# CristianSimion5/vk-raytracing-engine

Measured on AMD Instinct MI355X. Metric: Mrays/s, higher is better.
Workload: dtype f32

## Files before the change

vk-raytracing-engine_amd/csrc/traverse_share.h:

```cpp
#pragma once
#include "traverse_wide.h"

#define VKRT_SHARE_LDS_WORDS 384
struct ShareRes
{
  unsigned long long* key;
  int* slot;
  float* u;
  float* v;
  int* donor;
};
VKRT_DEV void shareSync()
{
  __builtin_amdgcn_fence(__ATOMIC_RELEASE, "wavefront");
  __builtin_amdgcn_wave_barrier();
  __builtin_amdgcn_fence(__ATOMIC_ACQUIRE, "wavefront");
}
VKRT_DEV unsigned laneRank(unsigned long long mask)
{
  return __builtin_amdgcn_mbcnt_hi((unsigned)(mask >> 32), __builtin_amdgcn_mbcnt_lo((unsigned)mask, 0u));
}
typedef unsigned vkrt_u32x2 __attribute__((ext_vector_type(2)));
typedef __attribute__((address_space(3))) vkrt_u32x2* ShareStk;
VKRT_DEV uint2 stkLoad(ShareStk p)
{
  const vkrt_u32x2 e = *p;
  return make_uint2(e.x, e.y);
}
VKRT_DEV void stkStore(ShareStk p, uint2 e)
{
  vkrt_u32x2 w;
  w.x = e.x; w.y = e.y;
  *p = w;
}
VKRT_DEV ShareRes shareRes(int* lds320)
{
  ShareRes r;
  r.key = (unsigned long long*)lds320; r.slot = lds320 + 128; r.u = (float*)(lds320 + 192); r.v = (float*)(lds320 + 256); r.donor = lds320 + 320;
  return r;
}

template <bool COUNT, bool ANYHIT, int TM = 0>
VKRT_DEV void traverse_wide8_share(const DevScene& sc, bool valid, f3 o, f3 d, float tmin, float tmax, uint2* stk, ShareRes res, RayHit& hit,
                                   TravCount& tc, uint32_t raySeed = 0u)
{
  TriRay<(TM & VKRT_TM_WATERTIGHT) != 0> tr;
  tr.set(d);
  const float4* __restrict__ nodes = sc.nodes;
  const float4* __restrict__ tris = sc.tris;
  const int stride = 64;
  const int lane = (int)lane_id();
  const ShareStk stkBase = (ShareStk)stk, stkCap = stkBase + (int)(sc.stackCap >> 1) * stride;
  const unsigned shareMin = sc.shareMinIdle;
  bool farFirst = ANYHIT && anyhit_far_first(sc, o, d, tmax);

  res.key[lane] = ((unsigned long long)__float_as_uint(tmax) << 32) | 0xffffffffull;
  res.slot[lane] = -1; res.u[lane] = 0.0f; res.v[lane] = 0.0f;
  shareSync();

  int owner = lane;
  unsigned long long* ownerKey = res.key + lane;
  int* ownerSlot = res.slot + lane;
  f3 id = mk3(safe_inv(d.x), safe_inv(d.y), safe_inv(d.z));
  bool px = !(id.x < 0.0f), py = !(id.y < 0.0f), pz = !(id.z < 0.0f);
  unsigned oct4 = ((px ? 1u : 0u) | (py ? 2u : 0u) | (pz ? 4u : 0u)) * 0x01010101u;
  uint2 G = make_uint2(0u, (valid && sc.rootRef != VKRT_TRAV_DONE) ? 0x80000000u : 0u);
  uint2 T = make_uint2(0u, 0u);
  ShareStk sp = stkBase, sb = stkBase, top = stkCap;
  bool busy = G.y != 0u;
  const unsigned iterLimit = sc.stepLimit > 0x03ffffffu ? 0xffffffffu : sc.stepLimit * 64u;
  const bool lendOn = (TM & (VKRT_TM_WATERTIGHT | VKRT_TM_DISSOLVE)) != (VKRT_TM_WATERTIGHT | VKRT_TM_DISSOLVE) && (sc.shareFlags & VKRT_SHARE_TRI_LEND) != 0u;

  for(unsigned iter = 0;; iter++)
  {
    const unsigned long long busyMask = __ballot(busy);
    if(busyMask == 0ull || iter >= iterLimit)
      break;
    if((iter & sc.sharePeriodMask) == sc.sharePeriodMask && (unsigned)__popcll(~busyMask) >= shareMin)
    {
      const bool giveStack = busy && sp > sb;
      const bool giveChild = (sc.shareFlags & 1u) != 0u && busy && !giveStack && (G.y & 0xff000000u & ((G.y & 0xff000000u) - 1u)) != 0u;
      const bool mayTris = (sc.shareFlags & 16u) != 0u && busy && !giveStack && !giveChild;
      const bool giveParked = mayTris && top < stkCap;
      const bool giveTris = mayTris && !giveParked && (T.y & (T.y - 1u)) != 0u;
      const bool wants = giveStack || giveChild || giveParked || giveTris;
      const unsigned long long donorMask = __ballot(wants), idleMask = ~busyMask;
      if(donorMask != 0ull)
      {
        const unsigned n = min((unsigned)__popcll(donorMask), (unsigned)__popcll(idleMask));
        const unsigned giveRank = laneRank(donorMask), takeRank = laneRank(idleMask);
        const bool gives = wants && giveRank < n;
        const bool takes = !busy && takeRank < n;
        uint2 e = make_uint2(0u, 0u);
        if(gives)
        {
          if(giveStack)
          {
            e = stkLoad(sb);
            sb += stride;
          }
          else if(giveChild)
          {
            const unsigned top = G.y & 0xff000000u;
            const unsigned low = farFirst ? (0x80000000u >> (unsigned)__clz((int)top)) : (top & (0u - top));
            e = make_uint2(G.x, low | (G.y & 0xffu));
            G.y &= ~low;
          }
          else if(giveParked)
          {
            e = stkLoad(top);
            e.x |= 0x80000000u;
            top += stride;
          }
          else
          {
            const unsigned lo = (unsigned)__ffs((int)T.y) - 1u, hi = 31u - (unsigned)__clz((int)T.y);
            const unsigned upper = T.y & ~((1u << ((lo + hi + 1u) >> 1)) - 1u);
            e = make_uint2(T.x | 0x80000000u, upper);
            T.y &= ~upper;
          }
          res.donor[giveRank] = lane;
        }
        shareSync();
        const int src = takes ? res.donor[takeRank] : lane;
        const unsigned ex = (unsigned)__shfl((int)e.x, src), ey = (unsigned)__shfl((int)e.y, src);
        const float ox = __shfl(o.x, src), oy = __shfl(o.y, src), oz = __shfl(o.z, src);
        const float dx = __shfl(d.x, src), dy = __shfl(d.y, src), dz = __shfl(d.z, src);
        const float ix = __shfl(id.x, src), iy = __shfl(id.y, src), iz = __shfl(id.z, src);
        const float tm = __shfl(tmax, src);
        const int ow = __shfl(owner, src);
        const unsigned o4 = (unsigned)__shfl((int)oct4, src);
        if(TM & VKRT_TM_DISSOLVE)
        {
          const uint32_t sd = (uint32_t)__shfl((int)raySeed, src);
          if(takes) raySeed = sd;
        }
        if(takes)
        {
          o = mk3(ox, oy, oz); d = mk3(dx, dy, dz); id = mk3(ix, iy, iz); tmax = tm;
          tr.set(d);
          farFirst = ANYHIT && anyhit_far_first(sc, o, d, tmax);
          px = !(id.x < 0.0f); py = !(id.y < 0.0f); pz = !(id.z < 0.0f);
          oct4 = o4;
          if(ex & 0x80000000u)
          {
            G = make_uint2(0u, 0u);
            T = make_uint2(ex & 0x7fffffffu, ey);
          }
          else
          {
            G = make_uint2(ex, ey);
            T = make_uint2(0u, 0u);
          }
          sp = stkBase; sb = stkBase; top = stkCap;
          owner = ow;
          ownerKey = res.key + ow; ownerSlot = res.slot + ow;
          busy = true;
        }
      }
    }
    shareSync();
    if(busy || lendOn)
    {
      float bt = tmax;
      int bg = -1;
      bool finished = false;
      bool occluded = false;
      if(ANYHIT)
        finished = busy && __hip_atomic_load(ownerSlot, __ATOMIC_RELAXED, __HIP_MEMORY_SCOPE_WAVEFRONT) >= 0;
      else
      {
        const unsigned long long k = __hip_atomic_load(ownerKey, __ATOMIC_RELAXED, __HIP_MEMORY_SCOPE_WAVEFRONT);
        bt = __uint_as_float((unsigned)(k >> 32));
        bg = (int)(unsigned)k;
      }
      if(!finished)
      {
        struct Cand
        {
          bool found;
          float t, u, v;
          int slot, gid;
        };
        auto testOne = [&](Cand& cd) {
          const unsigned i = (unsigned)__ffs((int)T.y) - 1u;
          T.y &= T.y - 1u;
          const unsigned s = T.x + i;
          const float4* __restrict__ tp = tris + (size_t)s * VKRT_TRI_QUADS;
          const float4 a = tp[0];
          const float4 b = tp[1];
          const float4 c = tp[2];
          if(COUNT)
          {
            tc.tris++;
            if(lane == __ffsll((long long)__ballot(1)) - 1) tc.waveTriSteps++;
          }
          float t, u, v;
          bool ccw;
          if(tr.hit(o, d, a, b, c, t, u, v, ccw) && t > tmin)
          {
            if(ANYHIT)
            {
              if(t < tmax && !cd.found && !query_rejects<TM>(sc, c, ccw) && !anyhit_ignores<TM>(sc, s, c.y, raySeed, VKRT_HOOK_UV(TM, u, v)))
              {
                cd.found = true; cd.t = t; cd.slot = (int)s;
              }
            }
            else
            {
              const int gid = tri_gid<TM>(c.y);
              const float rt = cd.found ? cd.t : bt;
              const int rg = cd.found ? cd.gid : bg;
              if((t < rt || (t == rt && gid < rg)) && !query_rejects<TM>(sc, c, ccw) && !anyhit_ignores<TM>(sc, s, c.y, raySeed, VKRT_HOOK_UV(TM, u, v)))
              {
                cd.found = true; cd.t = t; cd.u = u; cd.v = v; cd.slot = (int)s; cd.gid = gid;
              }
            }
          }
        };
        auto publish = [&](const Cand& cd) {
          if(!cd.found)
            return;
          if(ANYHIT)
          {
            __hip_atomic_store(ownerSlot, cd.slot, __ATOMIC_RELAXED, __HIP_MEMORY_SCOPE_WAVEFRONT);
            occluded = true;
          }
          else
          {
            const unsigned long long mine = ((unsigned long long)__float_as_uint(cd.t) << 32) | (unsigned)cd.gid;
            __hip_atomic_fetch_min(ownerKey, mine, __ATOMIC_RELAXED, __HIP_MEMORY_SCOPE_WAVEFRONT);
            shareSync();
            if(__hip_atomic_load(ownerKey, __ATOMIC_RELAXED, __HIP_MEMORY_SCOPE_WAVEFRONT) == mine)
            {
              res.slot[owner] = cd.slot; res.u[owner] = cd.u; res.v[owner] = cd.v;
            }
            bt = cd.t; bg = cd.gid;
          }
        };
        auto flushT = [&]() {
          Cand cd = {false, 0.0f, 0.0f, 0.0f, -1, 0};
          while(T.y != 0u && !(ANYHIT && cd.found))
            testOne(cd);
          publish(cd);
        };
        if(G.y & 0xff000000u)
        {
          const unsigned bitIdx = farFirst ? (unsigned)__ffs((int)(G.y & 0xff000000u)) - 1u : 31u - (unsigned)__clz((int)G.y);
          const unsigned slot = (bitIdx - 24u) ^ (oct4 & 7u);
          const unsigned child = G.x + (unsigned)__popc(G.y & 0xffu & ((1u << slot) - 1u));
          G.y &= ~(1u << bitIdx);
          if(G.y & 0xff000000u)
          {
            bool full = sp >= top;
            if(__builtin_expect(full && top < stkCap - VKRT_W8_POSTPONE_ROOM * stride, 0))
            {
              const uint2 keep = T;
              T = stkLoad(top);
              top += stride;
              flushT();
              T = keep;
              full = sp >= top;
            }
            if(!full)
            {
              stkStore(sp, G);
              sp += stride;
            }
            else
              VKRT_TRAV_FAULT(sc);
          }
          uint2 Tn;
          w8_test_children<COUNT, (TM & VKRT_TM_FILTER) != 0>(nodes, child, o, id, oct4, px, py, pz, tmin, bt, G, Tn, tc, query_node_masks<TM>(sc),
                                                              query_cull_mask<TM>(sc));
          if(Tn.y != 0u)
          {
            if(T.y != 0u)
            {
              if(__builtin_expect(top > stkCap - VKRT_W8_MAX_POSTPONED * stride && sp < top, 1))
              {
                top -= stride;
                stkStore(top, T);
              }
              else
              {
                if(!occluded)
                  flushT();
                T.y = 0u;
              }
            }
            T = Tn;
          }
        }
        if((G.y & 0xff000000u) == 0u && sp > sb)
        {
          sp -= stride;
          G = stkLoad(sp);
        }
        if(T.y == 0u && top < stkCap)
        {
          T = stkLoad(top);
          top += stride;
        }
        const unsigned long long hasTMask = __ballot(T.y != 0u);
        bool triStep = true;
        if(sc.triThreshold > 1u)
          triStep = (unsigned)__popcll(hasTMask) * 64u >= sc.triThreshold * (unsigned)__popcll(busyMask) ||
                    __ballot((G.y & 0xff000000u) != 0u) == 0ull;
        bool lentStep = false;
        if(lendOn && triStep)
        {
          const bool tests = T.y != 0u && !occluded;
          const unsigned rest1 = T.y & (T.y - 1u);
          const bool multi = rest1 != 0u && !occluded, isFree = T.y == 0u && !occluded;
          const unsigned long long lendMask = __ballot(multi), freeMask = ANYHIT ? __ballot(isFree) : (__ballot(true) & ~hasTMask);
          const unsigned n = min((unsigned)__popcll(lendMask), (unsigned)__popcll(freeMask));
          if(n != 0u)
          {
            lentStep = true;
            const unsigned lendRank = laneRank(lendMask), freeRank = laneRank(freeMask);
            const bool borrows = isFree && freeRank < n;
            unsigned s = 0u, ls = 0u;
            if(multi && lendRank < n)
            {
              const unsigned hi = 31u - (unsigned)__clz((int)T.y);
              T.y &= ~(1u << hi);
              ls = T.x + hi;
              res.donor[lendRank] = lane;
            }
            if(tests)
            {
              s = T.x + (unsigned)__ffs((int)T.y) - 1u;
              T.y &= T.y - 1u;
            }
            shareSync();
            const int src = borrows ? res.donor[freeRank] : lane;
            const unsigned bs = (unsigned)__shfl((int)ls, src);
            const f3 ro = mk3(__shfl(o.x, src), __shfl(o.y, src), __shfl(o.z, src));
            const f3 rd = mk3(__shfl(d.x, src), __shfl(d.y, src), __shfl(d.z, src));
            const int row = __shfl(owner, src);
            const float rbt = __shfl(bt, src);
            const int rbg = ANYHIT ? 0 : __shfl(bg, src);
            uint32_t rseed = raySeed;
            if(TM & VKRT_TM_DISSOLVE)
              rseed = (uint32_t)__shfl((int)raySeed, src);
            if(tests || borrows)
            {
              if(borrows)
              {
                s = bs;
                tr.set(rd);
              }
              const float4* __restrict__ tp = tris + (size_t)s * VKRT_TRI_QUADS;
              const float4 a = tp[0];
              const float4 b = tp[1];
              const float4 c = tp[2];
              if(COUNT)
              {
                tc.tris++;
                if(lane == __ffsll((long long)__ballot(1)) - 1) tc.waveTriSteps++;
              }
              float t, u, v;
              bool ccw;
              if(tr.hit(ro, rd, a, b, c, t, u, v, ccw) && t > tmin)
              {
                if(ANYHIT)
                {
                  if(t < rbt && !query_rejects<TM>(sc, c, ccw) && !anyhit_ignores<TM>(sc, s, c.y, rseed, VKRT_HOOK_UV(TM, u, v)))
                  {
                    __hip_atomic_store(&res.slot[row], (int)s, __ATOMIC_RELAXED, __HIP_MEMORY_SCOPE_WAVEFRONT);
                    if(!borrows)
                      occluded = true;
                  }
                }
                else
                {
                  const int gid = tri_gid<TM>(c.y);
                  if((t < rbt || (t == rbt && gid < rbg)) && !query_rejects<TM>(sc, c, ccw) && !anyhit_ignores<TM>(sc, s, c.y, rseed, VKRT_HOOK_UV(TM, u, v)))
                  {
                    const unsigned long long mine = ((unsigned long long)__float_as_uint(t) << 32) | (unsigned)gid;
                    __hip_atomic_fetch_min(&res.key[row], mine, __ATOMIC_RELAXED, __HIP_MEMORY_SCOPE_WAVEFRONT);
                    shareSync();
                    if(__hip_atomic_load(&res.key[row], __ATOMIC_RELAXED, __HIP_MEMORY_SCOPE_WAVEFRONT) == mine)
                    {
                      res.slot[row] = (int)s; res.u[row] = u; res.v[row] = v;
                    }
                  }
                }
              }
              if((TM & VKRT_TM_WATERTIGHT) != 0 && borrows)
                tr.set(d);
            }
          }
        }
        if(!lentStep && T.y != 0u && triStep && !occluded)
        {
          Cand cd = {false, 0.0f, 0.0f, 0.0f, -1, 0};
          testOne(cd);
          publish(cd);
        }
        if(ANYHIT && occluded)
          finished = true;
        else if((G.y & 0xff000000u) == 0u && T.y == 0u && top == stkCap)
          finished = true;
      }
      if(finished)
      {
        if(lendOn && busy)
        {
          G.y = 0u; T.y = 0u; sp = stkBase; sb = stkBase; top = stkCap;
        }
        busy = false;
      }
    }
  }
  if(__builtin_expect(busy, 0))
    VKRT_TRAV_FAULT(sc);
  shareSync();
  hit.t = __uint_as_float((unsigned)(res.key[lane] >> 32)); hit.u = res.u[lane]; hit.v = res.v[lane]; hit.slot = res.slot[lane];
  if(ANYHIT)
    hit.t = tmax;
}
```

vk-raytracing-engine_amd/csrc/vkrt_api.cpp:

```cpp
#include <hip/hip_runtime.h>

#include <algorithm>
#include <chrono>
#include <cmath>
#include <cstdarg>
#include <cstdio>
#include <cstdlib>
#include <cstring>
#include <initializer_list>
#include <string>
#include <vector>

#include "../../include/vkrt.h"
#include "bvh_host.h"
#include "dev_buffer.h"
#include "device_scene.h"
#include "kernels.h"
#include "scene_options.h"
#include "scene_pack.h"
#include "wide_node.h"

#include "lbvh.h"
#include "morph.h"
#include "refit.h"
#include "skin.h"
#include "vertex_update.h"

namespace {

thread_local std::string g_lastError;

int fail(int code, const char* fmt, ...)
{
  char buf[512];
  va_list ap;
  va_start(ap, fmt);
  vsnprintf(buf, sizeof buf, fmt, ap);
  va_end(ap);
  g_lastError = buf;
  return code;
}

#define HIP_TRY(expr)                                                      \
  do                                                                       \
  {                                                                        \
    std::string m_;                                                        \
    if(const int rc_ = vkrt::hip_status((expr), #expr, m_); rc_ != VKRT_OK) \
      return fail(rc_, "%s", m_.c_str());                                  \
  } while(0)

}

struct vkrt_scene
{
  int device = 0;
  int cuCount = 256;
  std::vector<float> positions;
  std::vector<uint32_t> indices;
  std::vector<vkrt_prim_mesh> primMeshes;
  std::vector<vkrt_node> nodes;
  uint32_t lightCount = 0, materialCount = 0;
  std::vector<float> materialAlpha;
  vkrt::DevArena tables;
  DevScene dev{};
  vkrt::TreeBuffers accel;
  bool built = false;
  vkrt_accel_info info{};
  unsigned int* workCounter = nullptr;
  DevCounters* counters = nullptr;
  vkrt::DevEvent evStart, evStop;
  bool timed = false;
  vkrt::DevBuf wfMem;
  WfBuffers wf{};
  vkrt::DevStream wfStreams[VKRT_WF_MAX_LANES];
  vkrt::DevEvent wfFork, wfJoin[VKRT_WF_MAX_LANES];
  WfAsync wfAsync{};
  std::vector<vkrt::DevEvent> wfEventOwners;
  std::vector<hipEvent_t> wfEvents;
  WfTiming wfTiming{};
  bool wfTimed = false;
  int splitResolved = 0;
  int wfTimingRounds = 0;
  std::vector<vkrt::DevEvent> wfPoolOwners;
  std::vector<hipEvent_t> wfPool;
  int opt[vkrt::kOptionLast + 1];
  bool hasLargeTriangles = false;
  bool wavefront = true;
  bool stale = false;
  bool refitted = false;
  vkrt::RefitScratch refit;
  bool positionsOnDevice = false;
  vkrt::DevBuf vertexStage;
  size_t vertexStageBytes = 0;
  struct Skin
  {
    vkrt::DevBuf mem;
    vkrt::SkinArrays arrays;
    uint32_t jointCount = 0;
  };
  std::vector<Skin> skins;
  struct Morph
  {
    vkrt::DevBuf mem;
    vkrt::MorphArrays arrays;
    int skin = -1;
  };
  std::vector<Morph> morphs;
  std::vector<vkrt_instance_visibility> vis;
  uint64_t masksPresent[4] = {0, 0, 0, 0};
  vkrt::DevBuf nodeMasks;
  std::vector<vkrt_material_alpha> alpha;
  uint32_t alphaMasks = 0;
  const uint4* surfacePrimMeshes = nullptr;
  vkrt::DevBuf motion;
  const DevInstance* prevInstances() const { return motion.get() ? motion.get<const DevInstance>() : dev.instances; }
  const float* prevPositions() const { return motion.get() ? (const float*)(motion.get<const char>() + motionPositionsAt()) : dev.positions; }
  size_t motionPositionsAt() const { return std::max<size_t>(nodes.size() * sizeof(DevInstance), 16); }
};

namespace {

template <typename T>
int upload(vkrt_scene* s, const T* src, size_t count, const T** dst)
{
  T* p = nullptr;
  HIP_TRY(s->tables.alloc(&p, count));
  if(count)
    HIP_TRY(hipMemcpy(p, src, count * sizeof(T), hipMemcpyHostToDevice));
  *dst = p;
  return VKRT_OK;
}

int failWith(int code, const std::string& err) { return fail(code, "%s", err.c_str()); }

bool useWavefront(const vkrt_scene* s) { return s->opt[VKRT_OPT_MODE] == 1; }

void freeAccel(vkrt_scene* s)
{
  s->accel = vkrt::TreeBuffers{};
  s->nodeMasks = vkrt::DevBuf{};
  s->built = false;
  s->refit = vkrt::RefitScratch{};
  s->refitted = false;
  s->stale = false;
}

void noteMasks(vkrt_scene* s)
{
  memset(s->masksPresent, 0, sizeof s->masksPresent);
  for(const vkrt_instance_visibility& v : s->vis)
    s->masksPresent[v.mask >> 6] |= 1ull << (v.mask & 63u);
}

bool everyMaskMeets(const vkrt_scene* s, uint32_t cullMask)
{
  for(uint32_t m = 0; m < 256; m++)
    if(((s->masksPresent[m >> 6] >> (m & 63u)) & 1ull) && (m & cullMask) == 0u)
      return false;
  return true;
}

int computeNodeMasks(vkrt_scene* s, hipStream_t stream)
{
  if(s->dev.layout != 1u || !s->nodeMasks.get())
    return VKRT_OK;
  const uint32_t nodes = (uint32_t)(s->info.node_bytes / VKRT_WNODE_BYTES);
  HIP_TRY(vkrt_launch_node_masks(s->dev, nodes, (uint32_t)s->nodes.size(), s->info.max_depth + 1u, s->nodeMasks.get<uint2>(), stream));
  return VKRT_OK;
}

int setDevice(const vkrt_scene* s)
{
// ... 284 lines not shown
  if(ndev <= 0)
    return fail(VKRT_ERR_NO_DEVICE, "no HIP device available (this library has no CPU path)");
  if(device < 0 || device >= ndev)
    return fail(VKRT_ERR_INVALID_ARGUMENT, "device %d out of range [0,%d)", device, ndev);
  vkrt_scene* s = new vkrt_scene();
  s->device = device;
  vkrt::initial_options(s->opt);
  auto bail = [&](int code) {
    vkrt_scene_destroy(s);
    return code;
  };
  if((rc = setDevice(s)) != VKRT_OK)
    return bail(rc);
  hipDeviceProp_t prop;
  if(hipGetDeviceProperties(&prop, device) == hipSuccess)
    s->cuCount = prop.multiProcessorCount;

  s->positions.assign(d->positions, d->positions + 3 * (size_t)d->vertex_count);
  s->indices.assign(d->indices, d->indices + d->index_count);
  s->primMeshes.assign(d->prim_meshes, d->prim_meshes + d->prim_mesh_count);
  s->nodes.assign(d->nodes, d->nodes + d->node_count);
  s->lightCount = d->light_count;
  s->materialCount = d->material_count;
  s->alpha.assign(d->material_count, vkrt::kDefaultAlpha);
  for(uint32_t i = 0; i < d->material_count; i++)
    s->materialAlpha.push_back(d->materials[i].pbrBaseColorFactor[3]);
  s->vis.assign(d->node_count, vkrt::kDefaultVisibility);
  noteMasks(s);

  const char* quadEnv = getenv("VKRT_TEX_QUADS");
  vkrt::PackedScene packed;
  if((rc = vkrt::pack_scene(d, !(quadEnv && atoi(quadEnv) == 0), packed, err)) != VKRT_OK)
    return bail(failWith(rc, err));
  DevScene& D = s->dev;
  const float *pn = nullptr, *lut = nullptr;
  const uint32_t *pm = nullptr, *quads = nullptr;
  if((rc = upload(s, d->positions, 3 * (size_t)d->vertex_count, &D.positions)) != VKRT_OK) return bail(rc);
  if((rc = upload(s, d->indices, (size_t)d->index_count, &D.indices)) != VKRT_OK) return bail(rc);
  if((rc = upload(s, packed.vertexPN.data(), packed.vertexPN.size(), &pn)) != VKRT_OK) return bail(rc);
  if((rc = upload(s, d->lights, (size_t)d->light_count, &D.lights)) != VKRT_OK) return bail(rc);
  if((rc = upload(s, packed.primMeshes.data(), packed.primMeshes.size(), &pm)) != VKRT_OK) return bail(rc);
  if((rc = upload(s, packed.instances.data(), packed.instances.size(), &D.instances)) != VKRT_OK) return bail(rc);
  if((rc = upload(s, packed.materials.data(), packed.materials.size(), &D.materials)) != VKRT_OK) return bail(rc);
  if((rc = upload(s, packed.shadeMaterials.data(), packed.shadeMaterials.size(), &D.shadeMaterials)) != VKRT_OK) return bail(rc);
  if((rc = upload(s, packed.textures.data(), packed.textures.size(), &D.textures)) != VKRT_OK) return bail(rc);
  if((rc = upload(s, packed.texMips.data(), packed.texMips.size(), &D.texMips)) != VKRT_OK) return bail(rc);
  if((rc = upload(s, packed.texels.data(), packed.texels.size(), &D.texels)) != VKRT_OK) return bail(rc);
  if(!packed.texQuads.empty() && (rc = upload(s, packed.texQuads.data(), packed.texQuads.size(), &quads)) != VKRT_OK) return bail(rc);
  if((rc = upload(s, packed.srgbLut, 512, &lut)) != VKRT_OK) return bail(rc);
  D.vertexPN = (const float4*)pn;
  s->surfacePrimMeshes = (const uint4*)pm;
  D.texQuads = (const uint4*)quads;
  D.srgbLut = lut;
  D.textureCount = d->texture_count;
  D.rootRef = VKRT_TRAV_DONE;
  D.stackCap = 1;
  D.layout = 0;
  D.stepLimit = 64;
  D.triThreshold = 0;
  D.shareMinIdle = 0;
  D.sharePeriodMask = 0;
  D.shareFlags = 0;
  D.gbufferMips = 1;

  if(s->tables.alloc(&s->workCounter, 16) != hipSuccess) return bail(fail(VKRT_ERR_OUT_OF_MEMORY, "hipMalloc(work counter)"));
  if(s->tables.alloc(&s->counters, 1) != hipSuccess) return bail(fail(VKRT_ERR_OUT_OF_MEMORY, "hipMalloc(counters)"));
  D.faults = &s->counters->v[0][10];
  if(hipMemset(s->counters, 0, sizeof(DevCounters)) != hipSuccess) return bail(fail(VKRT_ERR_HIP, "hipMemset(counters)"));
  if(s->evStart.create() != hipSuccess || s->evStop.create() != hipSuccess)
    return bail(fail(VKRT_ERR_HIP, "hipEventCreate"));
  *out = s;
  return VKRT_OK;
}

void vkrt_scene_destroy(vkrt_scene* s)
{
  if(!s)
    return;
  (void)hipSetDevice(s->device);
  delete s;
}

int vkrt_scene_set_option(vkrt_scene* s, int option, int value)
{
  if(!s)
    return fail(VKRT_ERR_INVALID_ARGUMENT, "scene is NULL");
  if(option < VKRT_OPT_MODE || option > VKRT_OPT_ALPHA_TEST)
    return fail(VKRT_ERR_INVALID_ARGUMENT, "unknown option %d", option);
  if(vkrt::clamp_option(option, value) != value)
    return fail(VKRT_ERR_INVALID_ARGUMENT, "option %d: value %d out of range", option, value);
  s->opt[option] = value;
  if(option == VKRT_OPT_WF_TRI_LEND && s->built && s->dev.layout == 1u)
    s->dev.shareFlags = (s->dev.shareFlags & ~VKRT_SHARE_TRI_LEND) | (value ? VKRT_SHARE_TRI_LEND : 0u);
  return VKRT_OK;
}

int vkrt_scene_get_option(const vkrt_scene* s, int option, int* value)
{
  if(!s || !value)
    return fail(VKRT_ERR_INVALID_ARGUMENT, "NULL argument");
  if(option == VKRT_INFO_ANYHIT_ORDER)
  {
    *value = s->built ? (int)(s->dev.shareFlags & 6u) : 0;
    return VKRT_OK;
  }
  if(option == VKRT_INFO_SPLIT_BUDGET)
  {
    *value = s->built ? s->splitResolved : 0;
    return VKRT_OK;
  }
  if(option < VKRT_OPT_MODE || option > VKRT_OPT_ALPHA_TEST)
    return fail(VKRT_ERR_INVALID_ARGUMENT, "unknown option %d", option);
  *value = s->opt[option];
  return VKRT_OK;
}

int vkrt_reserve(vkrt_scene* s, const vkrt_shard* shard, void* hip_stream)
{
  if(!s)
    return fail(VKRT_ERR_INVALID_ARGUMENT, "NULL argument");
  return vkrt_reserve_frames(s, shard, (uint32_t)std::max(1, s->opt[VKRT_OPT_WF_FRAMES_IN_FLIGHT]), hip_stream);
}

int vkrt_reserve_frames(vkrt_scene* s, const vkrt_shard* shard, uint32_t frames_per_call, void* hip_stream)
{
  if(!s || !shard)
    return fail(VKRT_ERR_INVALID_ARGUMENT, "NULL argument");
  if(frames_per_call == 0)
    return fail(VKRT_ERR_INVALID_ARGUMENT, "frames_per_call is 0");
  int rc = checkShard(shard);
  if(rc == VKRT_OK)
    rc = setDevice(s);
  if(rc != VKRT_OK)
    return rc;
  uint32_t tiles = 0;
  if((rc = shardTiles(shard, tiles)) != VKRT_OK)
    return rc;
  const bool wavefront = s->built ? s->wavefront : useWavefront(s);
  if(tiles == 0 || !wavefront)
    return VKRT_OK;
  return ensureFrameCall(s, tiles, frames_per_call, (hipStream_t)hip_stream);
}

namespace {

void installTree(vkrt_scene* s, vkrt::BuiltTree& t)
{
  s->accel = std::move(t.buf);
  s->dev.nodes = s->accel.nodes.get<const float4>();
  s->dev.tris = s->accel.tris.get<const float4>();
  s->dev.triShade = s->accel.triShade.get<const uint4>();
  s->dev.layout = t.layout;
  s->dev.rootRef = t.rootRef;
  s->dev.stackCap = t.layout == 1 ? 2 * (t.maxDepth + 1) : t.maxDepth + 2;
  s->info.node_count = t.nodeCount;
  s->info.max_depth = t.maxDepth;
  s->info.sah_cost = t.sahCost;
  s->info.node_bytes = t.nodeBytes;
  s->info.triangle_bytes = t.triangleBytes;
}

int uploadHostTree(vkrt_scene* s, const std::vector<vkrt::FlatTri>& tris, const vkrt::BuiltBvh* bvh, const vkrt::BuiltWide8* w8,
                   const std::vector<uint8_t>* instDissolves, hipStream_t stream, vkrt::BuiltTree& t)
{
  const std::vector<uint32_t>& order = w8 ? w8->triOrder : bvh->triOrder;
  std::vector<float> packed;
  std::vector<uint32_t> shadeRec;
  vkrt::pack_triangles(tris, order, packed, s->dev.watertight != 0, instDissolves);
  vkrt::pack_tri_shade(tris, order, s->indices.data(), s->primMeshes.data(), s->nodes.data(), shadeRec);
  const void* nodeData = w8 ? (const void*)w8->nodes.data() : (const void*)bvh->nodes.data();
  t = w8 ? vkrt::BuiltTree{1, tris.empty() ? VKRT_TRAV_DONE : 0, w8->maxDepth, w8->nodeCount, w8->sahCost, w8->nodes.size() * 4, packed.size() * 4}
         : vkrt::BuiltTree{0, bvh->rootRef, bvh->maxDepth, (uint32_t)(bvh->nodes.size() / 16), bvh->sahCost, bvh->nodes.size() * 4, packed.size() * 4};
  hipError_t e = hipSuccess;
  auto tryHip = [&](hipError_t x) { if(e == hipSuccess) e = x; };
  tryHip(t.buf.nodes.alloc(std::max<size_t>(t.nodeBytes, VKRT_WNODE_MIN_ALLOC)));
  tryHip(t.buf.tris.alloc(std::max<size_t>(t.triangleBytes, 48)));
  tryHip(t.buf.triShade.alloc(std::max<size_t>(shadeRec.size() * 4, 16)));
  if(e == hipSuccess && t.nodeBytes) tryHip(hipMemcpyAsync(t.buf.nodes.get(), nodeData, t.nodeBytes, hipMemcpyHostToDevice, stream));
  if(e == hipSuccess && !packed.empty()) tryHip(hipMemcpyAsync(t.buf.tris.get(), packed.data(), t.triangleBytes, hipMemcpyHostToDevice, stream));
  if(e == hipSuccess && !shadeRec.empty()) tryHip(hipMemcpyAsync(t.buf.triShade.get(), shadeRec.data(), shadeRec.size() * 4, hipMemcpyHostToDevice, stream));
  if(e == hipSuccess) tryHip(hipStreamSynchronize(stream));
  std::string m;
  const int rc = vkrt::hip_status(e, "uploading the acceleration structure", m);
  return rc == VKRT_OK ? VKRT_OK : fail(rc, "%s", m.c_str());
}

int traversalSettings(vkrt_scene* s)
{
  s->info.reference_count = s->dev.triCount;
  s->dev.stepLimit = 4u * (s->info.node_count + s->dev.triCount) + 64u;
  s->dev.triThreshold = 0;
  s->dev.shareMinIdle = 0;
  s->dev.sharePeriodMask = 0;
  s->dev.shareFlags = (uint32_t)s->opt[VKRT_OPT_WF_SHARE_FLAGS] & 6u;
  const bool largeWhole = s->hasLargeTriangles && s->info.reference_count == s->info.triangle_count;
  if((s->opt[VKRT_OPT_WF_SHARE_FLAGS] & 8) && !largeWhole)
    s->dev.shareFlags |= 4u;
  if(s->dev.layout == 1)
  {
    s->dev.triThreshold = (uint32_t)s->opt[VKRT_OPT_TRI_THRESHOLD];
    if(s->dev.triThreshold != 0u)
      s->dev.stackCap += 2 * VKRT_W8_POSTPONE_ROOM;
    s->dev.shareMinIdle = (uint32_t)s->opt[VKRT_OPT_WF_SHARE];
    s->dev.sharePeriodMask = (uint32_t)s->opt[VKRT_OPT_WF_SHARE_PERIOD];
    s->dev.shareFlags |= (uint32_t)s->opt[VKRT_OPT_WF_SHARE_FLAGS] & 17u;
    if(s->opt[VKRT_OPT_WF_TRI_LEND])
      s->dev.shareFlags |= VKRT_SHARE_TRI_LEND;
  }
  if((size_t)s->dev.stackCap * 256 * 4 > 64 * 1024)
    return fail(VKRT_ERR_UNSUPPORTED, "BVH depth %u needs a %zu-byte LDS stack per workgroup (limit 64 KiB)", s->info.max_depth,
                (size_t)s->dev.stackCap * 256 * 4);
  return VKRT_OK;
}

int accelBuildOnce(vkrt_scene* s, uint32_t flags, int splitBudget, hipStream_t stream)
{
  if(flags == 0)
    flags = VKRT_BUILD_DEFAULT;
  const bool wantPloc = (flags & VKRT_BUILD_PLOC_GPU) != 0;
  const bool wantLbvh = (flags & VKRT_BUILD_LBVH_GPU) != 0 || wantPloc, wantSah = (flags & VKRT_BUILD_SAH_HOST) != 0;
  if(wantLbvh == wantSah || (wantPloc && (flags & VKRT_BUILD_LBVH_GPU) != 0) || (flags & ~7u) != 0)
    return fail(VKRT_ERR_INVALID_ARGUMENT, "build_flags must select exactly one of VKRT_BUILD_LBVH_GPU / VKRT_BUILD_PLOC_GPU / VKRT_BUILD_SAH_HOST");
  int rc = setDevice(s);
  if(rc != VKRT_OK)
    return rc;
  HIP_TRY(hipStreamSynchronize(stream));
  freeAccel(s);
  const auto t0 = std::chrono::steady_clock::now();
  s->info = vkrt_accel_info{};
  s->info.build_flags = wantPloc ? VKRT_BUILD_PLOC_GPU : wantLbvh ? VKRT_BUILD_LBVH_GPU : VKRT_BUILD_SAH_HOST;
  s->wavefront = useWavefront(s);
  const bool watertight = s->opt[VKRT_OPT_WATERTIGHT] != 0;
  if((watertight || s->opt[VKRT_OPT_ANYHIT_DISSOLVE] != 0) && useWavefront(s) && s->opt[VKRT_OPT_WF_TRAV_BLOCK] != 64)
    return fail(VKRT_ERR_UNSUPPORTED, "VKRT_OPT_WATERTIGHT / VKRT_OPT_ANYHIT_DISSOLVE are built for the default 64-thread traversal workgroups "
                "(VKRT_OPT_WF_TRAV_BLOCK = %d)", s->opt[VKRT_OPT_WF_TRAV_BLOCK]);
  std::vector<uint8_t> instDissolves;
  bool dissolve = false;
  if(s->opt[VKRT_OPT_ANYHIT_DISSOLVE] != 0)
    for(const vkrt_node& n : s->nodes)
    {
      const int32_t m = std::max(0, s->primMeshes[(size_t)n.primMesh].materialIndex);
      const bool nonOpaque = s->materialAlpha[(size_t)m] < 1.0f && s->primMeshes[(size_t)n.primMesh].indexCount >= 3u;
      instDissolves.push_back(nonOpaque ? 1 : 0);
      dissolve = dissolve || nonOpaque;
    }
  s->dev.watertight = watertight ? 1u : 0u;
  s->dev.dissolve = dissolve ? 1u : 0u;
  const std::vector<uint8_t>* dissolvePtr = dissolve ? &instDissolves : nullptr;
  const bool wide = useWavefront(s) && s->opt[VKRT_OPT_BVH_LAYOUT] == 1;

  vkrt::BuiltTree tree;
  if(wantSah)
  {
    std::vector<vkrt::FlatTri> tris;
    vkrt::flatten_instances(s->positions.data(), s->indices.data(), s->primMeshes.data(), s->nodes.data(),
                            (uint32_t)s->nodes.size(), tris);
    vkrt::BuiltBvh bvh;
    vkrt::BuiltWide8 w8;
    if(wide)
      vkrt::build_wide8_host(tris, w8, watertight);
    else
      vkrt::build_sah_host(tris, 4, bvh, watertight);
    if((rc = uploadHostTree(s, tris, wide ? nullptr : &bvh, wide ? &w8 : nullptr, dissolvePtr, stream, tree)) != VKRT_OK)
      return rc;
    s->dev.triCount = (uint32_t)tris.size();
    s->info.triangle_count = (uint32_t)tris.size();
  }
  else
  {
    vkrt::LbvhParams p;
    p.wide = wide;
    p.ploc = wantPloc;
    p.splitPercent = (unsigned)splitBudget;
    vkrt::LbvhResult r;
    rc = vkrt::build_lbvh_device(s->dev, (uint32_t)s->nodes.size(), s->primMeshes, s->nodes, p, stream, r);
    if(rc != VKRT_OK)
      return fail(rc, "%s build failed: %s", wantPloc ? "PLOC" : "LBVH", r.error.c_str());
    s->info.triangle_count = r.uniqueTris;
    s->dev.triCount = r.triCount;
    if(r.wide.buf.nodes.get())
      tree = std::move(r.wide);
    else if(wide && r.triCount > 0)
    {
      vkrt::BuiltBvh b2;
      b2.nodes.resize((size_t)r.tree.nodeCount * 16);
      std::vector<float> records((size_t)r.triCount * 12);
      hipError_t e = hipSuccess;
      if(r.tree.nodeCount) e = hipMemcpy(b2.nodes.data(), r.tree.buf.nodes.get(), b2.nodes.size() * 4, hipMemcpyDeviceToHost);
      if(e == hipSuccess) e = hipMemcpy(records.data(), r.tree.buf.tris.get(), records.size() * 4, hipMemcpyDeviceToHost);
      r.tree.buf = vkrt::TreeBuffers{};
      if(e != hipSuccess)
        return fail(VKRT_ERR_HIP, "LBVH download: %s", hipGetErrorString(e));
      b2.rootRef = r.tree.rootRef;
      b2.maxDepth = r.tree.maxDepth;
      b2.triOrder.resize(r.triCount);
      std::vector<vkrt::FlatTri> tris(r.triCount);
      for(uint32_t k = 0; k < r.triCount; k++)
      {
        b2.triOrder[k] = k;
        tris[k] = vkrt::unpack_triangle(&records[(size_t)k * 12], watertight);
      }
      vkrt::BuiltWide8 w8;
      vkrt::collapse_wide8(b2, tris, w8, watertight);
      if((rc = uploadHostTree(s, tris, nullptr, &w8, dissolvePtr, stream, tree)) != VKRT_OK)
        return rc;
    }
    else
      tree = std::move(r.tree);
  }
  installTree(s, tree);
  vkrt::scene_bounds(s->positions, s->indices, s->primMeshes, s->nodes, s->dev.sceneLo, s->dev.sceneHi, s->hasLargeTriangles);
  if((rc = traversalSettings(s)) != VKRT_OK)
    return rc;
  if(s->dev.layout == 1u)
  {
    HIP_TRY(s->nodeMasks.alloc(std::max<size_t>(s->info.node_bytes / VKRT_WNODE_BYTES * 8, 16)));
    if((rc = computeNodeMasks(s, stream)) != VKRT_OK)
      return rc;
  }
  s->info.build_ms = std::chrono::duration<float, std::milli>(std::chrono::steady_clock::now() - t0).count();
  s->built = true;
  return VKRT_OK;
}

}

int vkrt_accel_build(vkrt_scene* s, uint32_t flags, void* hip_stream)
{
  if(!s)
    return fail(VKRT_ERR_INVALID_ARGUMENT, "scene is NULL");
  hipStream_t stream = (hipStream_t)hip_stream;
  if(s->positionsOnDevice)
  {
    int rc = setDevice(s);
    if(rc != VKRT_OK)
      return rc;
    HIP_TRY(hipDeviceSynchronize());
    if(!s->positions.empty())
      HIP_TRY(hipMemcpy(s->positions.data(), s->dev.positions, s->positions.size() * sizeof(float), hipMemcpyDeviceToHost));
    s->positionsOnDevice = false;
  }
  const bool deviceBuild = flags == 0 || (flags & (VKRT_BUILD_LBVH_GPU | VKRT_BUILD_PLOC_GPU)) != 0;
  if(s->opt[VKRT_OPT_SPLIT_BUDGET] >= 0 || !deviceBuild)
  {
    s->splitResolved = std::max(0, s->opt[VKRT_OPT_SPLIT_BUDGET]);
    return accelBuildOnce(s, flags, s->splitResolved, stream);
  }
  const auto t0 = std::chrono::steady_clock::now();
  float sahSplit = 0.0f;
  int rc = accelBuildOnce(s, flags, 30, stream);
  if(rc == VKRT_OK)
  {
    sahSplit = s->info.sah_cost;
    rc = accelBuildOnce(s, flags, 0, stream);
  }
// ... 1327 lines not shown
```

vk-raytracing-engine_amd/csrc/wf_traverse.hip:

```cpp
#include <hip/hip_runtime.h>

#include "device_math.h"
#include "device_scene.h"
#include "kernels.h"
#include "rgen.h"
#include "traverse.h"
#include "traverse_wide.h"
#include "traverse_share.h"
#include "wf_streams.h"

enum { WF_K_CLOSEST_C = 0, WF_K_CLOSEST_P = 1, WF_K_SHADOW_S = 2, WF_K_SHADOW_P = 3 };

VKRT_DEV void storeHit(const TraceParams& P, const WfBuffers& B, int par, int kind, unsigned qi, const RayHit& hit)
{
  if(kind == WF_K_SHADOW_S)
    wfStore(rec(B, par, WF_S, WF_H0, qi), make_float4(0.0f, 0.0f, 0.0f, __int_as_float(hit.slot >= 0 ? 0 : -1)));
  else if(kind == WF_K_SHADOW_P)
    ((float*)rec(B, par, WF_P, WF_H0, qi))[0] = __int_as_float(hit.slot >= 0 ? 1 : 0);
  else
  {
    const int type = kind == WF_K_CLOSEST_C ? WF_C : WF_P;
    int inst = -1;
    if(hit.slot >= 0)
    {
      const uint4 ts = P.sc.triShade[hit.slot];
      inst = __float_as_int(P.sc.tris[hit.slot * VKRT_TRI_QUADS + 2].z);
      wfStore(rec(B, par, type, WF_H1, qi), make_float4(__uint_as_float(ts.x), __uint_as_float(ts.y), __uint_as_float(ts.z), __uint_as_float(ts.w)));
    }
    float* h = (float*)rec(B, par, type, WF_H0, qi);
    if(type == WF_C)
      wfStore(rec(B, par, WF_C, WF_H0, qi), make_float4(hit.t, hit.u, hit.v, __int_as_float(inst)));
    else
    {
      h[1] = hit.u; h[2] = hit.v; h[3] = __int_as_float(inst);
    }
  }
}

template <bool COUNT, bool WIDE, int TB, int TM = 0>
__global__ __launch_bounds__(TB)
__attribute__((amdgpu_waves_per_eu(TM != 0 && WIDE && TB == 64 ? (COUNT && (TM & VKRT_TM_ALPHA) != 0 ? 4 : 5) : 1)))
void k_wf_traverse(const TraceParams P, const WfBuffers B, const int round)
{
  extern __shared__ int lds_stack[];
  const int par = round & 1;
  const unsigned cC = *countOf(B, par, WF_C), cS = *countOf(B, par, WF_S), cP = *countOf(B, par, WF_P);
  if(blockIdx.x == 0 && threadIdx.x == 0)
  {
    for(int t = 0; t < WF_TYPES; t++) *countOf(B, par ^ 1, t) = 0u;
    if(cC + cP) atomicAdd(&P.counters->v[round % VKRT_COUNTER_SLOTS][0], (unsigned long long)cC + cP);
    if(cS + cP) atomicAdd(&P.counters->v[round % VKRT_COUNTER_SLOTS][1], (unsigned long long)cS + cP);
    if(cP) atomicAdd(&P.counters->v[round % VKRT_COUNTER_SLOTS][11], (unsigned long long)cP);
  }
  const unsigned nC = (cC + TB - 1) / TB, nP = (cP + TB - 1) / TB, nS = (cS + TB - 1) / TB;
  unsigned blk = blockIdx.x;
  int kind;
  unsigned count;
  if(blk < nC) { kind = WF_K_CLOSEST_C; count = cC; }
  else if((blk -= nC) < nP) { kind = WF_K_CLOSEST_P; count = cP; }
  else if((blk -= nP) < nS) { kind = WF_K_SHADOW_S; count = cS; }
  else if((blk -= nS) < nP) { kind = WF_K_SHADOW_P; count = cP; }
  else return;
  const bool anyHit = kind >= WF_K_SHADOW_S;
  const int type = kind == WF_K_CLOSEST_C ? WF_C : kind == WF_K_SHADOW_S ? WF_S : WF_P;
  const unsigned qi = blk * TB + threadIdx.x;
  const bool valid = qi < count;
  float4 r0 = make_float4(0.0f, 0.0f, 0.0f, 0.0f), r1 = make_float4(1.0f, 0.0f, 0.0f, 0.0f);
  if(valid)
  {
    r0 = wfLoad(rec(B, par, type, WF_R0, qi));
    r1 = wfLoad(rec(B, par, type, kind == WF_K_CLOSEST_P ? WF_R2 : WF_R1, qi));
    if(kind == WF_K_CLOSEST_P)
      r0.w = 10000.0f;
  }
  uint32_t raySeed = 0u;
  if((TM & VKRT_TM_DISSOLVE) && valid)
    raySeed = __float_as_uint(wfLoad(rec(B, par, type, WF_S0, qi)).w);
  TravCount tc;
  __shared__ int shareLds[VKRT_SHARE_LDS_WORDS];
  RayHit hit;
  if(WIDE && TB == 64 && P.sc.shareMinIdle != 0u && P.sc.triThreshold != 0u)
  {
    uint2* stk = ((uint2*)lds_stack) + threadIdx.x;
    if(anyHit)
      traverse_wide8_share<COUNT, true, TM>(P.sc, valid, mk3(r0.x, r0.y, r0.z), mk3(r1.x, r1.y, r1.z), 0.001f, r0.w, stk, shareRes(shareLds), hit, tc, raySeed);
    else
      traverse_wide8_share<COUNT, false, TM>(P.sc, valid, mk3(r0.x, r0.y, r0.z), mk3(r1.x, r1.y, r1.z), 0.001f, r0.w, stk, shareRes(shareLds), hit, tc, raySeed);
    if(valid)
      storeHit(P, B, par, kind, qi, hit);
  }
  else if(valid)
  {
    traverse_any<COUNT, WIDE, TM>(P.sc, mk3(r0.x, r0.y, r0.z), mk3(r1.x, r1.y, r1.z), 0.001f, r0.w, anyHit, lds_stack, (int)threadIdx.x, TB, hit, tc, raySeed);
    storeHit(P, B, par, kind, qi, hit);
  }
  if(COUNT)
  {
    __shared__ unsigned long long red[VKRT_COUNTER_STRIDE * (TB / 64)];
    const unsigned vals[10] = {0, 0, 0, 0, 0, 0, tc.nodes, tc.tris, tc.waveNodeSteps, tc.waveTriSteps};
    blockAddCounters(&P.counters->v[blockIdx.x % VKRT_COUNTER_SLOTS][0], vals, 10, red);
  }
}

template <bool COUNT, int TM>
__global__ __launch_bounds__(64)
__attribute__((amdgpu_waves_per_eu(TM != 0 ? 5 : 1)))
void k_wf_traverse_camera(const TraceParams P, const WfBuffers B, const int round, const int smpl)
{
  extern __shared__ int lds_stack[];
  const int par = round & 1;
  if(blockIdx.x == 0 && threadIdx.x == 0)
    for(int t = 0; t < WF_TYPES; t++) *countOf(B, par ^ 1, t) = 0u;
  const unsigned w = blockIdx.x * 64u + threadIdx.x;
  uint32_t x = 0, y = 0, lrow = 0;
  const bool valid = pixelOfWork(P, w, P.tileFirst, x, y, lrow);
  f3 o = mk3(0.0f), d = mk3(1.0f, 0.0f, 0.0f);
  uint32_t raySeed = 0u;
  if(valid)
  {
    LaneState L;
    bindPixel(P, L, x, lrow);
    L.prd.seed = smpl == 0 ? pixelSeed(P, x, y) : __float_as_uint(((const float*)(B.sampleState + pixelSlot(P, x, lrow)))[3]);
    L.smpl = smpl;
    startSample(P, L);
    o = L.prd.rayOrigin; d = L.prd.rayDirection;
    raySeed = L.prd.seed;
  }
  const unsigned nValid = (unsigned)__popcll(__ballot(valid));
  if(threadIdx.x == 0 && nValid)
  {
    atomicAdd(&P.counters->v[blockIdx.x % VKRT_COUNTER_SLOTS][0], (unsigned long long)nValid);
    if(smpl == 0) atomicAdd(&P.counters->v[blockIdx.x % VKRT_COUNTER_SLOTS][5], (unsigned long long)nValid);
  }
  TravCount tc;
  __shared__ int shareLds[VKRT_SHARE_LDS_WORDS];
  RayHit hit;
  uint2* stk = ((uint2*)lds_stack) + threadIdx.x;
  traverse_wide8_share<COUNT, false, TM>(P.sc, valid, o, d, 0.001f, 10000.0f, stk, shareRes(shareLds), hit, tc, raySeed);
  if(valid)
    storeHit(P, B, par, WF_K_CLOSEST_C, w, hit);
  if(COUNT)
  {
    __shared__ unsigned long long red[VKRT_COUNTER_STRIDE];
    const unsigned vals[10] = {0, 0, 0, 0, 0, 0, tc.nodes, tc.tris, tc.waveNodeSteps, tc.waveTriSteps};
    blockAddCounters(&P.counters->v[blockIdx.x % VKRT_COUNTER_SLOTS][0], vals, 10, red);
  }
}

void vkrt_wf_launch_traverse(const TraceParams& P, const WfBuffers& B, int r, unsigned travBlock, bool count, dim3 tg, size_t tlds, hipStream_t stream)
{
  const bool wide = P.sc.layout == 1u;
  const dim3 tb(travBlock);
#define VKRT_TRAV_LAUNCH(C, W, TB, TM) hipLaunchKernelGGL((k_wf_traverse<C, W, TB, TM>), tg, tb, tlds, stream, P, B, r)
#define VKRT_TRAV_MODES(TB, TM)                                                                                                        \
  do {                                                                                                                                 \
    if(wide) { if(count) VKRT_TRAV_LAUNCH(true, true, TB, TM); else VKRT_TRAV_LAUNCH(false, true, TB, TM); }                           \
    else { if(count) VKRT_TRAV_LAUNCH(true, false, TB, TM); else VKRT_TRAV_LAUNCH(false, false, TB, TM); }                             \
  } while(0)
#define VKRT_TRAV_64(TM) VKRT_TRAV_MODES(64, TM)
  if(travBlock == 64)
  {
    VKRT_FRAME_TM_SWITCH(frame_tri_mode(P.sc, false), VKRT_TM_DISSOLVE, VKRT_TRAV_64)
  }
  else if(travBlock == 128)
    VKRT_TRAV_MODES(128, 0);
  else
    VKRT_TRAV_MODES(256, 0);
#undef VKRT_TRAV_64
#undef VKRT_TRAV_MODES
#undef VKRT_TRAV_LAUNCH
}

void vkrt_wf_launch_traverse_camera(const TraceParams& P, const WfBuffers& B, int r, int smpl, bool count, size_t tlds, hipStream_t stream)
{
#define VKRT_TRAV_CAMERA(TM)                                                                                                           \
  do {                                                                                                                                 \
    if(count) hipLaunchKernelGGL((k_wf_traverse_camera<true, TM>), dim3(P.tileCount), dim3(64), tlds, stream, P, B, r, smpl);          \
    else hipLaunchKernelGGL((k_wf_traverse_camera<false, TM>), dim3(P.tileCount), dim3(64), tlds, stream, P, B, r, smpl);              \
  } while(0)
  VKRT_FRAME_TM_SWITCH(frame_tri_mode(P.sc, false), VKRT_TM_DISSOLVE, VKRT_TRAV_CAMERA)
#undef VKRT_TRAV_CAMERA
}
```

Measured before the change: 5703.

## Replace LDS donor table with ds_permute routing and shrink shared LDS for occupancy

Result: faster. 5929, median of 6 (+4.0%).

```diff
diff --git a/vk-raytracing-engine_amd/csrc/trav_lds.h b/vk-raytracing-engine_amd/csrc/trav_lds.h
--- /dev/null
+++ b/vk-raytracing-engine_amd/csrc/trav_lds.h
@@ -0,0 +1,35 @@
+#pragma once
+#include <cstddef>
+#include <cstdint>
+
+#define VKRT_LDS_BYTES_PER_CU 163840u
+#define VKRT_LDS_GRANULE_BYTES 1280u
+#define VKRT_SIMDS_PER_CU 4u
+#define VKRT_SHARE_LDS_WORDS_SIX 320
+
+inline uint32_t travStackCap(uint32_t layout, uint32_t maxDepth, bool postpone, uint32_t postponeRoom)
+{
+  if(layout != 1u)
+    return maxDepth + 2u;
+  return 2u * (maxDepth + 1u) + (postpone ? 2u * postponeRoom : 0u);
+}
+
+struct TravLds
+{
+  size_t dynamicBytes;
+  size_t staticBytes;
+  size_t chargedBytes;
+  uint32_t wavesPerCu;
+  uint32_t wavesPerSimd;
+};
+
+inline TravLds travLdsPlan(uint32_t stackCap)
+{
+  TravLds p;
+  p.dynamicBytes = (size_t)stackCap * 64u * sizeof(uint32_t);
+  p.staticBytes = (size_t)VKRT_SHARE_LDS_WORDS_SIX * sizeof(uint32_t);
+  p.chargedBytes = (p.dynamicBytes + p.staticBytes + VKRT_LDS_GRANULE_BYTES - 1u) / VKRT_LDS_GRANULE_BYTES * VKRT_LDS_GRANULE_BYTES;
+  p.wavesPerCu = (uint32_t)(VKRT_LDS_BYTES_PER_CU / p.chargedBytes);
+  p.wavesPerSimd = p.wavesPerCu / VKRT_SIMDS_PER_CU < 6u ? p.wavesPerCu / VKRT_SIMDS_PER_CU : 6u;
+  return p;
+}
diff --git a/vk-raytracing-engine_amd/csrc/traverse_share.h b/vk-raytracing-engine_amd/csrc/traverse_share.h
--- a/vk-raytracing-engine_amd/csrc/traverse_share.h
+++ b/vk-raytracing-engine_amd/csrc/traverse_share.h
@@ -1,4 +1,5 @@
 #pragma once
+#include "trav_lds.h"
 #include "traverse_wide.h"
 
 #define VKRT_SHARE_LDS_WORDS 384
@@ -40,7 +41,14 @@
   return r;
 }
 
-template <bool COUNT, bool ANYHIT, int TM = 0>
+VKRT_DEV int laneOfRank(bool gives, unsigned giveRank, unsigned long long giveMask, unsigned takeRank, int lane)
+{
+  const unsigned slot = gives ? giveRank : (unsigned)__popcll(giveMask) + (unsigned)lane - giveRank;
+  const int byRank = __builtin_amdgcn_ds_permute((int)(slot << 2), lane);
+  return __builtin_amdgcn_ds_bpermute((int)(takeRank << 2), byRank);
+}
+
+template <bool COUNT, bool ANYHIT, int TM = 0, bool DONOR_LDS = true>
 VKRT_DEV void traverse_wide8_share(const DevScene& sc, bool valid, f3 o, f3 d, float tmin, float tmax, uint2* stk, ShareRes res, RayHit& hit,
                                    TravCount& tc, uint32_t raySeed = 0u)
 {
@@ -50,6 +58,7 @@
   const float4* __restrict__ tris = sc.tris;
   const int stride = 64;
   const int lane = (int)lane_id();
+  int* const donor = DONOR_LDS ? res.donor : (int*)res.u;
   const ShareStk stkBase = (ShareStk)stk, stkCap = stkBase + (int)(sc.stackCap >> 1) * stride;
   const unsigned shareMin = sc.shareMinIdle;
   bool farFirst = ANYHIT && anyhit_far_first(sc, o, d, tmax);
@@ -119,10 +128,20 @@
             e = make_uint2(T.x | 0x80000000u, upper);
             T.y &= ~upper;
           }
-          res.donor[giveRank] = lane;
-        }
-        shareSync();
-        const int src = takes ? res.donor[takeRank] : lane;
+          if(DONOR_LDS || ANYHIT)
+            donor[giveRank] = lane;
+        }
+        int src = lane;
+        if(DONOR_LDS || ANYHIT)
+        {
+          shareSync();
+          if(takes) src = donor[takeRank];
+        }
+        else
+        {
+          const int giver = laneOfRank(wants, giveRank, donorMask, takeRank, lane);
+          if(takes) src = giver;
+        }
         const unsigned ex = (unsigned)__shfl((int)e.x, src), ey = (unsigned)__shfl((int)e.y, src);
         const float ox = __shfl(o.x, src), oy = __shfl(o.y, src), oz = __shfl(o.z, src);
         const float dx = __shfl(d.x, src), dy = __shfl(d.y, src), dz = __shfl(d.z, src);
@@ -326,15 +345,25 @@
               const unsigned hi = 31u - (unsigned)__clz((int)T.y);
               T.y &= ~(1u << hi);
               ls = T.x + hi;
-              res.donor[lendRank] = lane;
+              if(DONOR_LDS || ANYHIT)
+                donor[lendRank] = lane;
             }
             if(tests)
             {
               s = T.x + (unsigned)__ffs((int)T.y) - 1u;
               T.y &= T.y - 1u;
             }
-            shareSync();
-            const int src = borrows ? res.donor[freeRank] : lane;
+            int src = lane;
+            if(DONOR_LDS || ANYHIT)
+            {
+              shareSync();
+              if(borrows) src = donor[freeRank];
+            }
+            else
+            {
+              const int lender = laneOfRank(multi, lendRank, lendMask, freeRank, lane);
+              if(borrows) src = lender;
+            }
             const unsigned bs = (unsigned)__shfl((int)ls, src);
             const f3 ro = mk3(__shfl(o.x, src), __shfl(o.y, src), __shfl(o.z, src));
             const f3 rd = mk3(__shfl(d.x, src), __shfl(d.y, src), __shfl(d.z, src));
@@ -417,7 +446,11 @@
   if(__builtin_expect(busy, 0))
     VKRT_TRAV_FAULT(sc);
   shareSync();
-  hit.t = __uint_as_float((unsigned)(res.key[lane] >> 32)); hit.u = res.u[lane]; hit.v = res.v[lane]; hit.slot = res.slot[lane];
+  int home = lane;
+  asm volatile("" : "+v"(home));
+  hit.t = __uint_as_float((unsigned)(res.key[home] >> 32)); hit.u = res.u[home]; hit.v = res.v[home]; hit.slot = res.slot[home];
   if(ANYHIT)
     hit.t = tmax;
-}
+  if(ANYHIT && !DONOR_LDS)
+    hit.u = 0.0f;
+}
diff --git a/vk-raytracing-engine_amd/csrc/vkrt_api.cpp b/vk-raytracing-engine_amd/csrc/vkrt_api.cpp
--- a/vk-raytracing-engine_amd/csrc/vkrt_api.cpp
+++ b/vk-raytracing-engine_amd/csrc/vkrt_api.cpp
@@ -18,6 +18,7 @@
 #include "kernels.h"
 #include "scene_options.h"
 #include "scene_pack.h"
+#include "trav_lds.h"
 #include "wide_node.h"
 
 #include "lbvh.h"
@@ -608,7 +609,7 @@
   s->dev.triShade = s->accel.triShade.get<const uint4>();
   s->dev.layout = t.layout;
   s->dev.rootRef = t.rootRef;
-  s->dev.stackCap = t.layout == 1 ? 2 * (t.maxDepth + 1) : t.maxDepth + 2;
+  s->dev.stackCap = travStackCap(t.layout, t.maxDepth, false, 0u);
   s->info.node_count = t.nodeCount;
   s->info.max_depth = t.maxDepth;
   s->info.sah_cost = t.sahCost;
@@ -655,8 +656,7 @@
   if(s->dev.layout == 1)
   {
     s->dev.triThreshold = (uint32_t)s->opt[VKRT_OPT_TRI_THRESHOLD];
-    if(s->dev.triThreshold != 0u)
-      s->dev.stackCap += 2 * VKRT_W8_POSTPONE_ROOM;
+    s->dev.stackCap = travStackCap(1u, s->info.max_depth, s->dev.triThreshold != 0u, VKRT_W8_POSTPONE_ROOM);
     s->dev.shareMinIdle = (uint32_t)s->opt[VKRT_OPT_WF_SHARE];
     s->dev.sharePeriodMask = (uint32_t)s->opt[VKRT_OPT_WF_SHARE_PERIOD];
     s->dev.shareFlags |= (uint32_t)s->opt[VKRT_OPT_WF_SHARE_FLAGS] & 17u;
diff --git a/vk-raytracing-engine_amd/csrc/wf_traverse.hip b/vk-raytracing-engine_amd/csrc/wf_traverse.hip
--- a/vk-raytracing-engine_amd/csrc/wf_traverse.hip
+++ b/vk-raytracing-engine_amd/csrc/wf_traverse.hip
@@ -39,7 +39,7 @@
 
 template <bool COUNT, bool WIDE, int TB, int TM = 0>
 __global__ __launch_bounds__(TB)
-__attribute__((amdgpu_waves_per_eu(TM != 0 && WIDE && TB == 64 ? (COUNT && (TM & VKRT_TM_ALPHA) != 0 ? 4 : 5) : 1)))
+__attribute__((amdgpu_waves_per_eu(WIDE && TB == 64 ? (TM == 0 ? (COUNT ? 1 : 6) : COUNT && (TM & VKRT_TM_ALPHA) != 0 ? 4 : 5) : 1)))
 void k_wf_traverse(const TraceParams P, const WfBuffers B, const int round)
 {
   extern __shared__ int lds_stack[];
@@ -65,32 +65,45 @@
   const int type = kind == WF_K_CLOSEST_C ? WF_C : kind == WF_K_SHADOW_S ? WF_S : WF_P;
   const unsigned qi = blk * TB + threadIdx.x;
   const bool valid = qi < count;
+  constexpr bool SHARING = WIDE && TB == 64;
   float4 r0 = make_float4(0.0f, 0.0f, 0.0f, 0.0f), r1 = make_float4(1.0f, 0.0f, 0.0f, 0.0f);
-  if(valid)
-  {
-    r0 = wfLoad(rec(B, par, type, WF_R0, qi));
-    r1 = wfLoad(rec(B, par, type, kind == WF_K_CLOSEST_P ? WF_R2 : WF_R1, qi));
-    if(kind == WF_K_CLOSEST_P)
-      r0.w = 10000.0f;
-  }
+  auto loadRay = [&]() {
+    if(valid)
+    {
+      r0 = wfLoad(rec(B, par, type, WF_R0, qi));
+      r1 = wfLoad(rec(B, par, type, kind == WF_K_CLOSEST_P ? WF_R2 : WF_R1, qi));
+      if(kind == WF_K_CLOSEST_P)
+        r0.w = 10000.0f;
+    }
+  };
+  if(!SHARING)
+    loadRay();
   uint32_t raySeed = 0u;
   if((TM & VKRT_TM_DISSOLVE) && valid)
     raySeed = __float_as_uint(wfLoad(rec(B, par, type, WF_S0, qi)).w);
   TravCount tc;
-  __shared__ int shareLds[VKRT_SHARE_LDS_WORDS];
+  __shared__ int shareLds[VKRT_SHARE_LDS_WORDS_SIX];
   RayHit hit;
   if(WIDE && TB == 64 && P.sc.shareMinIdle != 0u && P.sc.triThreshold != 0u)
   {
     uint2* stk = ((uint2*)lds_stack) + threadIdx.x;
     if(anyHit)
-      traverse_wide8_share<COUNT, true, TM>(P.sc, valid, mk3(r0.x, r0.y, r0.z), mk3(r1.x, r1.y, r1.z), 0.001f, r0.w, stk, shareRes(shareLds), hit, tc, raySeed);
+    {
+      loadRay();
+      traverse_wide8_share<COUNT, true, TM, false>(P.sc, valid, mk3(r0.x, r0.y, r0.z), mk3(r1.x, r1.y, r1.z), 0.001f, r0.w, stk, shareRes(shareLds), hit, tc, raySeed);
+    }
     else
-      traverse_wide8_share<COUNT, false, TM>(P.sc, valid, mk3(r0.x, r0.y, r0.z), mk3(r1.x, r1.y, r1.z), 0.001f, r0.w, stk, shareRes(shareLds), hit, tc, raySeed);
+    {
+      loadRay();
+      traverse_wide8_share<COUNT, false, TM, false>(P.sc, valid, mk3(r0.x, r0.y, r0.z), mk3(r1.x, r1.y, r1.z), 0.001f, r0.w, stk, shareRes(shareLds), hit, tc, raySeed);
+    }
     if(valid)
       storeHit(P, B, par, kind, qi, hit);
   }
   else if(valid)
   {
+    if(SHARING)
+      loadRay();
     traverse_any<COUNT, WIDE, TM>(P.sc, mk3(r0.x, r0.y, r0.z), mk3(r1.x, r1.y, r1.z), 0.001f, r0.w, anyHit, lds_stack, (int)threadIdx.x, TB, hit, tc, raySeed);
     storeHit(P, B, par, kind, qi, hit);
   }
@@ -104,7 +117,7 @@
 
 template <bool COUNT, int TM>
 __global__ __launch_bounds__(64)
-__attribute__((amdgpu_waves_per_eu(TM != 0 ? 5 : 1)))
+__attribute__((amdgpu_waves_per_eu(TM != 0 ? 5 : COUNT ? 1 : 6)))
 void k_wf_traverse_camera(const TraceParams P, const WfBuffers B, const int round, const int smpl)
 {
   extern __shared__ int lds_stack[];
@@ -133,10 +146,10 @@
     if(smpl == 0) atomicAdd(&P.counters->v[blockIdx.x % VKRT_COUNTER_SLOTS][5], (unsigned long long)nValid);
   }
   TravCount tc;
-  __shared__ int shareLds[VKRT_SHARE_LDS_WORDS];
+  __shared__ int shareLds[VKRT_SHARE_LDS_WORDS_SIX];
   RayHit hit;
   uint2* stk = ((uint2*)lds_stack) + threadIdx.x;
-  traverse_wide8_share<COUNT, false, TM>(P.sc, valid, o, d, 0.001f, 10000.0f, stk, shareRes(shareLds), hit, tc, raySeed);
+  traverse_wide8_share<COUNT, false, TM, false>(P.sc, valid, o, d, 0.001f, 10000.0f, stk, shareRes(shareLds), hit, tc, raySeed);
   if(valid)
     storeHit(P, B, par, WF_K_CLOSEST_C, w, hit);
   if(COUNT)
```
